# feinanshan/TDNet

Measured on AMD Instinct MI355X. Metric: frames/sec (td4-psp18, 1024x2048, full-resolution logits), higher is better.
Workload: dtype f32; 1 GPU; td4-psp18, 1024x2048 Cityscapes-shaped synthetic stream, 3-frame feature cache, 1 clip per GPU; parallelism=clip-parallel x1, RCCL weight broadcast only, target_fps_per_gpu=30

## Files before the change

include/tdnet.h:

```cpp
#ifndef TDNET_H
#define TDNET_H

#include <stddef.h>
#include <stdint.h>

#ifdef __cplusplus
extern "C" {
#endif

typedef struct tdnet tdnet_t;

typedef struct tdnet_cfg {
    int32_t model;
    int32_t backbone;
    int32_t nclass;
    int32_t height;
    int32_t width;
    int32_t device;
} tdnet_cfg;

#define TDNET_WINOGRAD_DEFAULT 3
#define TDNET_ATTENTION_DEFAULT 2
#define TDNET_FUSION_LN_STATS 2
#define TDNET_FUSION_LN_IN_HEAD 4
#define TDNET_FUSION_A_DIRECT 32
#define TDNET_FUSION_DMA_LOADERS 8192
#define TDNET_FUSION_DMA_NARROW 32768
#define TDNET_FUSION_STEM_ROWS 65536
#define TDNET_FUSION_CONV_GROUPS 131072
#define TDNET_FUSION_CLS_IN_HEAD 262144
#define TDNET_FUSION_SPLIT_NARROW 524288
#define TDNET_FUSION_LATE_CHAIN 1048576
#define TDNET_FUSION_PPM_FOLD 2097152
#define TDNET_OVERLAP_CHAINS 1
#define TDNET_OVERLAP_LOWREG_TRANSFORMS 2
#define TDNET_OVERLAP_CHAINS_ANY_SIZE 4
#define TDNET_OVERLAP_GEMM_DMA 8
#define TDNET_OVERLAP_VW_SHIFT 4
#define TDNET_OVERLAP_VW_MASK 0x30
#define TDNET_FUSION_DEFAULT (TDNET_FUSION_LN_STATS | TDNET_FUSION_LN_IN_HEAD | TDNET_FUSION_A_DIRECT | TDNET_FUSION_DMA_LOADERS | TDNET_FUSION_DMA_NARROW | \
                              TDNET_FUSION_STEM_ROWS | TDNET_FUSION_CONV_GROUPS | TDNET_FUSION_CLS_IN_HEAD | TDNET_FUSION_SPLIT_NARROW | TDNET_FUSION_LATE_CHAIN | TDNET_FUSION_PPM_FOLD)
#define TDNET_FUSION_MASK TDNET_FUSION_DEFAULT
#define TDNET_OVERLAP_DEFAULT (TDNET_OVERLAP_CHAINS | TDNET_OVERLAP_GEMM_DMA | (2 << TDNET_OVERLAP_VW_SHIFT))
#define TDNET_OVERLAP_MASK (TDNET_OVERLAP_CHAINS | TDNET_OVERLAP_LOWREG_TRANSFORMS | TDNET_OVERLAP_CHAINS_ANY_SIZE | TDNET_OVERLAP_GEMM_DMA | TDNET_OVERLAP_VW_MASK)
typedef struct tdnet_opts {
    int32_t winograd;
    int32_t precision;
    int32_t pipeline;
    int32_t gemm_persistent;
    int32_t reserved0;
    int32_t attention;
    int32_t fusion;
    int32_t overlap;
    int32_t reserved[8];
} tdnet_opts;
void tdnet_opts_default(tdnet_opts* o);

typedef struct tdnet_arch {
    int32_t dilated;
    int32_t multi_grid;
    int32_t reserved[6];
} tdnet_arch;
void tdnet_arch_default(tdnet_arch* a);

int  tdnet_create(const tdnet_cfg* cfg, tdnet_t** out);
int  tdnet_create_opts(const tdnet_cfg* cfg, const tdnet_opts* opts , tdnet_t** out);
int  tdnet_create_arch(const tdnet_cfg* cfg, const tdnet_arch* arch , const tdnet_opts* opts ,
                       tdnet_t** out);
int  tdnet_get_opts(const tdnet_t* h, tdnet_opts* out);
int  tdnet_get_arch(const tdnet_t* h, tdnet_arch* out);
int  tdnet_feature_dims(const tdnet_t* h, int* height, int* width);
void tdnet_destroy(tdnet_t* h);

int  tdnet_set_weight(tdnet_t* h, const char* name, const float* host, size_t count);
int  tdnet_finalize_weights(tdnet_t* h);
int  tdnet_create_shared(const tdnet_t* weights_of, const tdnet_opts* opts , tdnet_t** out);
int  tdnet_warmup(tdnet_t* h, void* stream);
// ... 81 lines not shown
```

tdnet_amd/_capi.py:

```python
import ctypes
import os

_HERE = os.path.dirname(os.path.abspath(__file__))
DEFAULT_LIB = os.path.join(_HERE, "lib", "libtdnet_hip.so")
TEST_LIB = os.path.join(_HERE, "lib", "libtdnet_hip_test.so")

c_float_p = ctypes.POINTER(ctypes.c_float)
c_void_p = ctypes.c_void_p


class TdnetCfg(ctypes.Structure):
    _fields_ = [("model", ctypes.c_int32), ("backbone", ctypes.c_int32), ("nclass", ctypes.c_int32),
                ("height", ctypes.c_int32), ("width", ctypes.c_int32), ("device", ctypes.c_int32)]


class TdnetOpts(ctypes.Structure):
    _fields_ = [("winograd", ctypes.c_int32), ("precision", ctypes.c_int32), ("pipeline", ctypes.c_int32),
                ("gemm_persistent", ctypes.c_int32), ("reserved0", ctypes.c_int32), ("attention", ctypes.c_int32),
                ("fusion", ctypes.c_int32), ("overlap", ctypes.c_int32), ("reserved", ctypes.c_int32 * 8)]

    def as_dict(self):
        return {k: getattr(self, k) for k, _ in self._fields_ if not k.startswith("reserved")}


# ... 106 lines not shown
    "tdnet_op_conv1x1_rows": (ctypes.c_int, [c_void_p, ctypes.c_int, ctypes.c_int, ctypes.c_int, c_void_p, c_void_p, ctypes.c_int, ctypes.c_int,
                                             c_opts_p, ctypes.c_int, ctypes.c_int, c_void_p, c_void_p]),
    "tdnet_op_maxpool": (ctypes.c_int, [c_void_p, ctypes.c_int, ctypes.c_int, ctypes.c_int, ctypes.c_int, c_void_p, c_void_p]),
    "tdnet_op_stem_f16": (ctypes.c_int, [c_void_p, ctypes.c_int, ctypes.c_int, c_void_p, c_void_p, ctypes.c_int, c_void_p, c_void_p]),
    "tdnet_op_stem": (ctypes.c_int, [c_void_p, ctypes.c_int, ctypes.c_int, c_void_p, c_void_p, c_opts_p, c_void_p, c_void_p]),
    "tdnet_op_attention": (ctypes.c_int, [c_void_p, c_void_p, c_void_p, c_void_p, c_void_p, ctypes.c_int, ctypes.c_int,
                                          ctypes.c_int, ctypes.c_int, c_void_p, c_void_p, c_void_p, c_void_p, c_void_p]),
    "tdnet_op_layernorm_hw": (ctypes.c_int, [c_void_p, ctypes.c_int, ctypes.c_int, c_void_p, c_void_p, c_void_p, c_void_p]),
    "tdnet_op_layernorm_hw_f16": (ctypes.c_int, [c_void_p, ctypes.c_int, ctypes.c_int, c_void_p, c_void_p, c_void_p, c_void_p]),
    "tdnet_op_ppm": (ctypes.c_int, [c_void_p, ctypes.c_int, ctypes.c_int, c_void_p, c_void_p, ctypes.c_int, ctypes.c_int,
                                    c_void_p, c_void_p]),
    "tdnet_op_upsample": (ctypes.c_int, [c_void_p, ctypes.c_int, ctypes.c_int, ctypes.c_int, ctypes.c_int, ctypes.c_int,
                                         c_void_p, c_void_p]),
    "tdnet_op_stem_image": (ctypes.c_long, [c_void_p, c_void_p, ctypes.c_int, ctypes.c_int, ctypes.c_int, ctypes.c_int, ctypes.POINTER(ctypes.c_double),
                                            ctypes.POINTER(ctypes.c_double), ctypes.c_int, c_void_p, ctypes.c_size_t, c_void_p]),
    "tdnet_op_stem_image_nv12": (ctypes.c_long, [c_void_p, ctypes.c_int, ctypes.c_int, ctypes.c_int, ctypes.c_size_t, ctypes.c_int, ctypes.c_int, ctypes.c_int,
                                                 ctypes.POINTER(ctypes.c_double), ctypes.POINTER(ctypes.c_double), ctypes.c_int, c_void_p, ctypes.c_size_t, c_void_p]),
    "tdnet_op_stem_image_view": (ctypes.c_long, [c_void_p, c_view_p, ctypes.c_int, ctypes.c_int, ctypes.POINTER(ctypes.c_double), ctypes.POINTER(ctypes.c_double),
                                                 ctypes.c_int, c_void_p, ctypes.c_size_t, c_void_p]),
    "tdnet_op_overlay_view": (ctypes.c_int, [c_void_p] + [ctypes.c_int] * 5 + [c_void_p, c_void_p, c_view_p, c_void_p, ctypes.c_int, c_void_p, c_void_p]),
    "tdnet_op_upsample_argmax": (ctypes.c_int, [c_void_p, ctypes.c_int, ctypes.c_int, ctypes.c_int, ctypes.c_int, ctypes.c_int, c_void_p, c_void_p, c_void_p]),
    "tdnet_op_upsample_argmax_rgb": (ctypes.c_int, [c_void_p] + [ctypes.c_int] * 7 + [c_void_p, ctypes.c_int, c_void_p, c_void_p, c_void_p]),
    "tdnet_op_overlay": (ctypes.c_int, [c_void_p] + [ctypes.c_int] * 5 + [c_void_p, c_void_p] + [ctypes.c_int] * 4 + [ctypes.c_size_t, ctypes.c_int, c_void_p, ctypes.c_int,
                                        c_void_p, c_void_p]),
    "tdnet_op_upsample_argmax_score": (ctypes.c_int, [c_void_p] + [ctypes.c_int] * 5 + [c_void_p] * 6),
    "tdnet_op_upsample_argmax_conf": (ctypes.c_int, [c_void_p] + [ctypes.c_int] * 5 + [c_void_p, c_void_p, ctypes.c_int, ctypes.c_int, c_void_p, c_void_p]),
    "tdnet_op_nearest_index": (ctypes.c_int, [ctypes.c_int, ctypes.c_int, c_void_p]),
    "tdnet_op_enc_first": (ctypes.c_int, [c_void_p] + [ctypes.c_int] * 4 + [c_void_p] * 4 + [ctypes.c_int] + [c_void_p] * 4 + [ctypes.c_int] + [c_void_p] * 5),
    "tdnet_op_conv1x1_src2_null": (ctypes.c_int, [c_void_p, ctypes.c_int, ctypes.c_int, ctypes.c_int, c_void_p, c_void_p, ctypes.c_int, ctypes.c_int,
                                                  c_void_p, ctypes.c_int, c_opts_p, ctypes.c_int, c_void_p, c_void_p]),
    "tdnet_op_classifier": (ctypes.c_int, [c_void_p, ctypes.c_int, ctypes.c_int, c_void_p, c_void_p, ctypes.c_int, c_void_p, c_void_p]),
    "tdnet_op_head_cls": (ctypes.c_int, [c_void_p, ctypes.c_int, ctypes.c_int, ctypes.c_int, c_void_p, c_void_p, ctypes.c_int, ctypes.c_int,
                                         c_void_p, c_void_p, ctypes.c_int, c_opts_p, ctypes.c_int, c_void_p, c_void_p]),
}


class Lib:

    def __init__(self, path=DEFAULT_LIB, test_symbols=False):
        if not os.path.exists(path):
            raise TdnetError("HIP library not found: %s -- build it with `python -c 'import __graft_entry__ as g; g.build()'` "
                             "(hipcc --offload-arch=gfx950); there is no CPU fallback" % path)
        self.path = path
        if path in (DEFAULT_LIB, TEST_LIB):
            import torch
        self.dll = ctypes.CDLL(path)
        for name, (res, args) in list(SYMBOLS.items()) + (list(TEST_SYMBOLS.items()) if test_symbols else []):
            fn = getattr(self.dll, name)
            fn.restype = res
            fn.argtypes = args
            setattr(self, name, fn)

    def opts(self, **kw):
        o = TdnetOpts()
        self.tdnet_opts_default(ctypes.byref(o))
        for k, v in kw.items():
            if k not in dict(TdnetOpts._fields_) or k.startswith("reserved"):
                raise TypeError("unknown tdnet_opts field %r" % k)
            if v is not None:
                setattr(o, k, int(v))
        return o

    def arch(self, dilated=True, multi_grid=True):
        a = TdnetArch()
        self.tdnet_arch_default(ctypes.byref(a))
        a.dilated, a.multi_grid = int(bool(dilated)), int(bool(multi_grid))
# ... 25 lines not shown
```

tdnet_amd/csrc/td_frame.h:

```cpp
#pragma once
#include "td_launch.h"

static int free_slot(tdnet* n) {
    for (int i = 0; i < (int)n->slots.size(); ++i) {
        bool used = i == n->pending_slot;
        for (int f : n->fifo) used |= f == i;
        if (!used) return i;
    }
    return -1;
}
static void fifo_commit(tdnet* n, int slot) {
    n->fifo.push_back(slot);
    if ((int)n->fifo.size() > n->FIFO) n->fifo.erase(n->fifo.begin());
    n->last_slot = slot;
}

static int launch_chain(tdnet* n, PathLayers& L, hipStream_t s, float* vp, int e0, int e1, int e2) {
    const int DV = n->DV;
    hipStream_t c = n->side;
    TD_HIP(hipEventRecord(n->ev_fork, s));
    TD_HIP(hipStreamWaitEvent(c, n->ev_fork, 0));
    if (probe_skip() & 2) { TD_HIP(hipEventRecord(n->ev_join, c)); return 0; }
    if (n->P == 4) {
        const CacheSlot &c0 = n->slots[e0], &c1 = n->slots[e1], &c2 = n->slots[e2];
        TD_TRY(run_conv(n, L.atn[0].fc, c0.v, 1, n->Lk, nullptr, vp, c));
        const bool sl = DV == 512 && n->Lk <= 8192;
        if (run_attention(n, c1.q, c0.k, vp, L.atn[0].d_bias, c1.v, n->Lk, n->Lk, DV, n->chain_a, c, n->opts.attention, nullptr, nullptr, sl)) return -1;
        TD_TRY(run_conv(n, L.atn[1].fc, n->chain_a, 1, n->Lk, nullptr, vp, c));
        if (run_attention(n, c2.q, c1.k, vp, L.atn[1].d_bias, c2.v, n->Lk, n->Lk, DV, n->chain_b, c, n->opts.attention, nullptr, nullptr, sl)) return -1;
        TD_TRY(run_conv(n, L.atn[2].fc, n->chain_b, 1, n->Lk, nullptr, vp, c));
    } else {
        TD_TRY(run_conv(n, L.atn[0].fc, n->slots[e0].v, 1, n->Lk, nullptr, vp, c));
    }
    if (n->vt16) {
        prof_begin(n, 2, false, 0, c);
        if (n->opts.precision >= 2) attn_prepare_vt_b3(vp, n->Lk, DV, reinterpret_cast<unsigned short*>(n->vt16), c);
        else attn_prepare_vt_h(vp, n->Lk, DV, n->vt16, c);
        prof_end(n, c);
    }
    TD_HIP(hipEventRecord(n->ev_join, c));
    return 0;
}
static int launch_chain_now(tdnet* n, PathLayers& L, hipStream_t s) {
    return launch_chain(n, L, s, n->vp, n->fifo[0], n->P == 4 ? n->fifo[1] : -1, n->P == 4 ? n->fifo[2] : -1);
}
static int run_ds_rows(tdnet* n, const ConvLayer& L, const float* in, int H, int W, float* out, int ny, int cy, hipStream_t s) {
    if (L.route != CR_GEMM1X1) return td_fail("internal: downsample conv cannot run on image rows");
// ... 62 lines not shown
        const bool last16 = n->act16 && &B == &L.blocks.back();
        if (B.bott) {
            TD_TRY(run_conv(n, B.c1, n->bx, ch, cw, nullptr, n->bt, s));
            TD_TRY(run_conv(n, B.c2, n->bt, ch, cw, nullptr, n->bu, s, &oh, &ow));
            const float* res = n->bx;
            if (B.has_ds) { TD_TRY(run_conv(n, B.ds, n->bx, ch, cw, nullptr, n->br, s)); res = n->br; }
            TD_TRY(run_conv(n, B.c3, n->bu, oh, ow, res, last16 ? n->br : n->bx, s));
        } else {
            const float* res = n->bx;
            if (B.has_ds) {
                const ConvCall both[2] = {{&B.c1, n->bx, ch, cw, n->bt}, {&B.ds, n->bx, ch, cw, n->br}};
                TD_TRY(run_conv_group(n, n->opts, both, 2, s, &oh, &ow));
                res = n->br;
            } else TD_TRY(run_conv(n, B.c1, n->bx, ch, cw, nullptr, n->bt, s, &oh, &ow));
            TD_TRY(run_conv(n, B.c2, n->bt, oh, ow, res, last16 ? n->br : n->bx, s));
        }
        ch = oh; cw = ow;
    }
    float* c4 = n->c4 = n->seg_block >= 0 ? n->seg_x.back() : n->act16 ? n->br : n->bx;
    if (n->cfg.model == 1) {
        run_ppm(n, c4, n->h, n->w, n->C, n->C, n->C / 4, L.d_ppm_w, L.d_ppm_b, 0, n->rowpart, n->pooled, n->ppmfeat, n->z, s);
        TD_TRY(run_conv(n, L.head3, n->z, n->h, n->w, nullptr, n->headmid, s));
        TD_TRY(run_classifier(n, n->headmid, n->Lq, n->MID, n->cfg.nclass, L.d_cls_w, L.d_cls_b, n->lowres, s));
        return n->failed ? -1 : 0;
    }
    const int XS = n->C / 2, FS = n->C / 8;
    const ConvLayer* const firstL[3] = {&L.enc_v, &L.enc_q0, &L.enc_k0};
    const PpmFoldArgs fold = n->enc_fold ? ppm_fold_args(firstL, n->fold_g, n->ppmfeat, XS, FS) : PpmFoldArgs();
    run_ppm(n, c4, n->h, n->w, n->C, XS, FS, L.d_ppm_w, L.d_ppm_b, L.pid, n->rowpart, n->pooled, n->ppmfeat, n->z, s, n->enc_fold ? &fold : nullptr);
    n->z_pending = n->enc_fold;
    n->z_path = (int)(&L - &n->paths[0]);
    const int slot = free_slot(n);
    if (slot < 0) return td_fail("internal: no free cache slot");
    CacheSlot& cs = n->slots[slot];
    const ConvCall first[3] = {{&L.enc_v, n->z, n->h, n->w, n->v_cur}, {&L.enc_q0, n->z, n->h, n->w, n->q1}, {&L.enc_k0, n->z, n->h, n->w, n->k1}};
    const ConvCall second[2] = {{&L.enc_q1, n->q1, n->h, n->w, n->q_cur}, {&L.enc_k1, n->k1, n->hk, n->wk, cs.k}};
    if (n->enc_fold) {
        float* const outs[3] = {n->v_cur, n->q1, n->k1};
        for (int i = 0; i < 3; ++i)
            TD_TRY(run_conv_src2(n, *firstL[i], c4 + L.pid * XS, n->C, XS / 32, XS / 32 + TD_PPM_BASIS / 32, n->ppm_basis, TD_PPM_BASIS, n->fold_g[i], n->h, n->w, nullptr, outs[i], s));
    } else
    TD_TRY(run_conv_group(n, n->opts, first, 3, s));
    TD_TRY(run_conv_group(n, n->opts, second, 2, s));
    prof_begin(n, 2, false, 0, s);
    launch_cache_subsample(n->q_cur, cs.q, 64, n->v_cur, cs.v, DV, n->w, n->hk, n->wk, s);
    prof_end(n, s);
    n->pending_slot = slot;
    return n->failed ? -1 : 0;
}

static int finish_frame(tdnet* n, PathLayers& L, bool steady, hipStream_t s) {
    const int DV = n->DV;
    const float* feat = n->v_cur;
    int stats_nstr = 0;
    n->feat_is_vcur = !steady;
    if (steady) {
        TD_HIP(hipStreamWaitEvent(s, n->ev_join, 0));
        const CacheSlot& ck = n->slots[n->fifo[n->FIFO - 1]];
        const AtnLayer& A = L.atn[n->P == 4 ? 2 : 0];
        stats_nstr = (n->opts.fusion & TDNET_FUSION_LN_STATS) ? attn_strips(n->Lq, DV) : 0;
        if (run_attention(n, n->q_cur, ck.k, n->vp, A.d_bias, n->v_cur, n->Lq, n->Lk, DV, n->feat, s, n->opts.attention,
                          stats_nstr ? n->ln_part : nullptr, nullptr, false, n->vt16 != nullptr, n->opts.precision >= 2)) return -1;
        feat = n->feat;
    }
    const bool ln_in_head = (n->opts.fusion & TDNET_FUSION_LN_IN_HEAD) && L.head3.wino;
    const bool ln16 = L.head3.in16;
    run_layernorm(n, feat, n->Lq, DV, L.d_ln_g, L.d_ln_b, n->ln_part, n->ln_mean, n->ln_rstd, ln_in_head ? nullptr : n->ln, s, stats_nstr, ln16);
    n->ln_pending = ln_in_head || ln16;
    n->ln_path = (int)(&L - &n->paths[0]);
    const bool cls_in_head = (n->opts.fusion & TDNET_FUSION_CLS_IN_HEAD) && L.head3.wino && L.head3.chunks == 1 && wino_out_cls_supports(n->MID, n->cfg.nclass);
    const ClsArgs ca = {L.d_cls_w, L.d_cls_b, n->lowres, n->cfg.nclass};
    if (ln_in_head) {
        const LnFuse lf = {n->ln_mean, n->ln_rstd, L.d_ln_g, L.d_ln_b};
        TD_TRY(run_conv(n, L.head3, feat, n->h, n->w, nullptr, n->headmid, s, nullptr, nullptr, &lf, cls_in_head ? &ca : nullptr));
    } else
    TD_TRY(run_conv(n, L.head3, n->ln, n->h, n->w, nullptr, n->headmid, s, nullptr, nullptr, nullptr, cls_in_head ? &ca : nullptr));
    if (!cls_in_head) TD_TRY(run_classifier(n, n->headmid, n->Lq, n->MID, n->cfg.nclass, L.d_cls_w, L.d_cls_b, n->lowres, s));
    if (n->failed) return -1;
    if (n->pending_slot >= 0) {
        const int slot = n->pending_slot;
        n->pending_slot = -1;
        fifo_commit(n, slot);
    }
    return 0;
}

static int frame_checks(tdnet* n, int pos_id, const char* who, const FrameInput* in = nullptr) {
    if (!n->finalized || !n->ws_ready) return td_fail("%s: weights not finalized (the HIP path never runs on random init)", who);
    if (in && in->kind == TD_IMG_U8 && !n->u8.set) return td_fail("%s: the uint8 input is not configured (call tdnet_set_input_u8 first)", who);
    if (pos_id < 0 || pos_id >= n->P) return td_fail("%s: pos_id %d out of range 0..%d", who, pos_id, n->P - 1);
    return 0;
}

static void rejoin_streams(tdnet* n, hipStream_t s) {
    for (hipStream_t c : {n->side, n->chain2}) {
        if (!c) continue;
        hipEvent_t& e = c == n->side ? n->ev_join : n->ev_cjoin;
        if (e && hipEventRecord(e, c) == hipSuccess) (void)hipStreamWaitEvent(s, e, 0);
    }
}

static int streams_share_a_queue(hipStream_t a, hipStream_t x, hipEvent_t e0, hipEvent_t e1, hipEvent_t e2, bool* shared) {
    float pair_us = 0.f;
    TD_HIP(td_streams_share_a_queue(a, x, e0, e1, e2, shared, &pair_us));
    if (getenv("TDNET_QUEUE_CHECK_VERBOSE")) fprintf(stderr, "tdnet queue check: spin pair %.1f us\n", pair_us);
    return 0;
}
static int place_chain_stream(tdnet* n, hipStream_t s, bool explicit_call = false) {
    if (!n->chain2 || std::find(n->placed_for.begin(), n->placed_for.end(), (void*)s) != n->placed_for.end()) return 0;
    if (!explicit_call && td_stream_is_capturing(s)) return 0;
    n->placed_for.push_back((void*)s);
    if (getenv("TDNET_NO_QUEUE_CHECK")) return 0;
    if (n->placed_for.size() > 8 || n->retired_streams.size() >= 12) return 0;
    hipEvent_t e0 = nullptr, e1 = nullptr, e2 = nullptr;
    TD_HIP(hipEventCreate(&e0)); TD_HIP(hipEventCreate(&e1)); TD_HIP(hipEventCreate(&e2));
    int rc = 0;
    for (int attempt = 0; attempt < 6 && n->retired_streams.size() < 12; ++attempt) {
        bool shared = false;
        if ((rc = streams_share_a_queue(s, n->chain2, e0, e1, e2, &shared)) != 0 || !shared) break;
        hipStream_t fresh = nullptr;
        if (hipStreamCreateWithFlags(&fresh, hipStreamNonBlocking) != hipSuccess) break;
        n->retired_streams.push_back(n->chain2);
        n->chain2 = fresh;
        n->chain_replaced++;
    }
    hipEventDestroy(e0); hipEventDestroy(e1); hipEventDestroy(e2);
    return rc;
// ... 28 lines not shown
```

tdnet_amd/csrc/td_handle.h:

```cpp
#pragma once
#include "../../include/tdnet.h"
#include "td_device.h"
#include "td_conv.h"
#include "td_conv_h.h"
#include "td_conv_hd.h"
#include "td_conv_ad.h"
#include "td_wino.h"
#include "td_gemm.h"
#include "td_gemm_dma.h"
#include "td_gemm_b3.h"
#include "td_conv_ad_b3.h"
#include "td_attn.h"
#include "td_attn_h.h"
#include "td_attn_b3.h"
#include "td_misc.h"
#include "td_ingest.h"
#include "td_out.h"
#include "td_score.h"
#include "td_conf.h"

#include <cmath>
#include <cstdarg>
#include <cstdio>
#include <algorithm>
// ... 89 lines not shown
    CR_STEM_H,
    CR_CONV_H,
    CR_CONV_DMA,
    CR_WINO
};
enum GemmKernel {
    GK_CONV,
    GK_PERSISTENT,
    GK_DMA,
    GK_B3
};
struct ConvLayer {
    int Cin = 0, Cout = 0, KS = 1, stride = 1, dil = 1, pad = 0, act = 0;
    bool stem = false;
    ConvRoute route = CR_IGEMM;
    GemmKernel gemm = GK_CONV;
    bool in16 = false, out16 = false;
    int rh = 0;
    bool rowimg_off = false;
    int pers = 1;
    int chunks = 1;
    int vw = 0;
    int wino = 0;
    float* d_zero = nullptr;
    ConvTile tile = CT_128x128;
    int CoutPad = 0, nsteps = 0;
    float* d_wp = nullptr;
    float* d_bias = nullptr;
    bool h16() const { return route == CR_STEM_H || route == CR_CONV_H || route == CR_CONV_DMA; }
    bool stem_rows() const { return route == CR_ADIRECT_ROWS || route == CR_ADIRECT_ROWS_B3; }
    double flops_per_pixel() const { return 2.0 * Cout * (stem ? 3.0 * KS * KS : (double)Cin * KS * KS); }
};

static_assert(TDNET_FUSION_DEFAULT == 4169766 && TDNET_FUSION_MASK == 4169766 && TDNET_OVERLAP_DEFAULT == 41 && TDNET_OVERLAP_MASK == 0x3f,
              "the named option bits of include/tdnet.h must add up to the documented values");
static tdnet_opts opts_or_default(const tdnet_opts* o) {
    tdnet_opts d;
    tdnet_opts_default(&d);
    if (!o) return d;
    d = *o;
    d.winograd = d.winograd <= 0 ? 0 : (d.winograd == 2 || d.winograd >= 4) ? 4 : 3;
    d.precision = d.precision < 0 ? 0 : d.precision > 3 ? 1 : d.precision;
    d.pipeline = d.pipeline ? 1 : 0;
    d.gemm_persistent = d.gemm_persistent < 0 ? 0 : d.gemm_persistent;
    d.attention = d.attention < 0 ? 0 : d.attention > 2 ? 2 : d.attention;
    d.fusion &= TDNET_FUSION_MASK;
    d.overlap = d.overlap < 0 ? 0 : d.overlap & TDNET_OVERLAP_MASK;
    if ((d.overlap & TDNET_OVERLAP_VW_MASK) == TDNET_OVERLAP_VW_MASK) d.overlap &= ~TDNET_OVERLAP_VW_MASK;
    d.reserved0 = 0;
    for (int& r : d.reserved) r = 0;
    return d;
}

struct BlockLayers { ConvLayer c1, c2, c3, ds; bool has_ds = false, bott = false; };
struct AtnLayer { ConvLayer fc; float* d_bias = nullptr; };
struct PathLayers {
    ConvLayer stem, stem2, stem3;
    std::vector<BlockLayers> blocks;
    float* d_ppm_w = nullptr; float* d_ppm_b = nullptr;
    ConvLayer enc_v, enc_q0, enc_q1, enc_k0, enc_k1;
    std::vector<AtnLayer> atn;
    float* d_ln_g = nullptr; float* d_ln_b = nullptr;
    ConvLayer head3;
    float* d_cls_w = nullptr; float* d_cls_b = nullptr;
    int pid = 0;
};
struct CacheSlot { float* q = nullptr; float* k = nullptr; float* v = nullptr; };
// ... 78 lines not shown
    tdnet_opts opts;
    int P = 0, DV = 0, MID = 0, FIFO = 0, C = 512, SC = 64;
    bool deep = false;
    int H = 0, W = 0, H1 = 0, W1 = 0, H2 = 0, W2 = 0, h = 0, w = 0, hk = 0, wk = 0, Lq = 0, Lk = 0;
    std::vector<BlockSpec>& bspec;
    std::map<std::string, std::vector<float>>& sd;
    std::map<std::string, size_t>& expected;
    bool& finalized;
    std::vector<PathLayers>& paths;
    int& seg_block; int& seg_conv;
    bool& act16;
    double& flops_frame;
    bool ws_ready = false;
    size_t ws_bytes = 0;
    float *img4 = nullptr, *s1 = nullptr, *s1b = nullptr, *bx = nullptr, *bt = nullptr, *br = nullptr, *bu = nullptr;
    float *rowpart = nullptr, *pooled = nullptr, *ppmfeat = nullptr, *z = nullptr;
    float *v_cur = nullptr, *q1 = nullptr, *q_cur = nullptr, *k1 = nullptr;
    float *vp = nullptr, *chain_a = nullptr, *chain_b = nullptr, *feat = nullptr;
    float *ln_part = nullptr, *ln_mean = nullptr, *ln_rstd = nullptr, *ln = nullptr;
    float *headmid = nullptr, *lowres = nullptr, *stage_tmp = nullptr, *logits_tmp = nullptr;
    float *wino_v = nullptr, *wino_m = nullptr;
    size_t wino_v_floats = 0, wino_m_floats = 0;
    size_t stage_tmp_floats = 0;
    std::vector<CacheSlot> slots;
    std::vector<int> fifo;
    int last_slot = -1;
    int pending_slot = -1;
    int pending_pos = -1;
    hipStream_t side = nullptr;
    hipEvent_t ev_fork = nullptr, ev_join = nullptr;
    hipStream_t chain2 = nullptr;
    hipEvent_t ev_cfork = nullptr, ev_cjoin = nullptr;
    float *wino_v2 = nullptr, *wino_m2 = nullptr;
    std::vector<float*> seg_t, seg_r, seg_x;
    std::vector<hipStream_t> probe_streams;
    std::vector<hipStream_t> retired_streams;
    std::vector<void*> placed_for;
    int chain_replaced = 0;
    float* c4 = nullptr;
    _Float16* vt16 = nullptr;
    bool ln_pending = false;
    bool enc_fold = false;
    float* ppm_basis = nullptr;
    float* fold_g[3] = {nullptr, nullptr, nullptr};
    bool z_pending = false;
    int z_path = 0;
    int ln_path = 0;
    bool feat_is_vcur = false;
    bool failed = false;
    bool prof = false;
    std::vector<ProfRec> recs;
    size_t nrec = 0;
    U8Input u8;
    RgbOutput rgb;
    OverlayOutput overlay;
    ScoreOutput score;
    int min_conf = 0, reject_label = 255;
    int launches = 0;

    explicit tdnet(TdWeights* w)
        : wt(w), bspec(w->bspec), sd(w->sd), expected(w->expected), finalized(w->finalized), paths(w->paths), seg_block(w->seg_block),
          seg_conv(w->seg_conv), act16(w->act16), flops_frame(w->flops_frame) {}
    tdnet(const tdnet&) = delete;
    tdnet& operator=(const tdnet&) = delete;
};

// ... 300 lines not shown
```

tdnet_amd/csrc/td_model.hip:

```cpp
#include "td_frame.h"

extern "C" const char* tdnet_last_error(void) { return g_err; }
#ifndef TDNET_SRC_HASH
#define TDNET_SRC_HASH "unstamped"
#endif
extern "C" const char* tdnet_version(void) { return "tdnet_amd 0.3 (gfx950, fp32 MFMA) tdnet-src-hash:" TDNET_SRC_HASH; }
extern "C" void tdnet_opts_default(tdnet_opts* o) {
    if (!o) return;
    memset(o, 0, sizeof(*o));
    o->winograd = TDNET_WINOGRAD_DEFAULT;
    o->precision = 0;
    o->pipeline = 1;
    o->gemm_persistent = 1;
    o->attention = TDNET_ATTENTION_DEFAULT;
    o->fusion = TDNET_FUSION_DEFAULT;
    o->overlap = TDNET_OVERLAP_DEFAULT;
}
extern "C" void tdnet_arch_default(tdnet_arch* a) {
    if (!a) return;
    memset(a, 0, sizeof(*a));
    a->dilated = 1;
    a->multi_grid = 1;
}
extern "C" int tdnet_create(const tdnet_cfg* cfg, tdnet_t** out) { return tdnet_create_opts(cfg, nullptr, out); }
// ... 83 lines not shown
    tdnet* n = new tdnet(weights_of->wt);
    n->wt->refs.fetch_add(1, std::memory_order_relaxed);
    set_geometry(n, &weights_of->cfg);
    n->opts = weights_of->opts;
    if (init_handle(n)) { tdnet_destroy(n); return -1; }
    *out = n;
    return 0;
}

extern "C" void tdnet_destroy(tdnet_t* n) {
    if (!n) return;
    TD_ON_DEVICE(n);
    for (float* q : {n->img4, n->s1, n->s1b, n->bx, n->bt, n->br, n->bu, n->rowpart, n->pooled, n->ppmfeat, n->z, n->v_cur, n->q1, n->q_cur,
                     n->k1, n->vp, n->chain_a, n->chain_b, n->feat, n->ln_part, n->ln_mean, n->ln_rstd, n->ln, n->headmid,
                     n->lowres, n->stage_tmp, n->logits_tmp, n->wino_v, n->wino_m, n->ppm_basis, n->fold_g[0], n->fold_g[1], n->fold_g[2]})
        if (q) hipFree(q);
    for (auto& s : n->slots) { if (s.q) hipFree(s.q); if (s.k) hipFree(s.k); if (s.v) hipFree(s.v); }
    for (auto& r : n->recs) { hipEventDestroy(r.e0); hipEventDestroy(r.e1); }
    if (n->vt16) hipFree(n->vt16);
    u8_free(n->u8);
    rgb_free(n->rgb);
    overlay_free(n->overlay);
    score_free(n->score);
    for (float* q : {n->wino_v2, n->wino_m2}) if (q) hipFree(q);
    for (auto* v : {&n->seg_t, &n->seg_r, &n->seg_x}) for (float* q : *v) if (q) hipFree(q);
    if (n->chain2) hipStreamDestroy(n->chain2);
    for (hipStream_t x : n->probe_streams) hipStreamDestroy(x);
    for (hipStream_t x : n->retired_streams) hipStreamDestroy(x);
    if (n->ev_cfork) hipEventDestroy(n->ev_cfork);
    if (n->ev_cjoin) hipEventDestroy(n->ev_cjoin);
    if (n->side) hipStreamDestroy(n->side);
    if (n->ev_fork) hipEventDestroy(n->ev_fork);
    if (n->ev_join) hipEventDestroy(n->ev_join);
    TdWeights* wt = n->wt;
    delete n;
    if (wt->refs.fetch_sub(1, std::memory_order_acq_rel) == 1) {
        for (auto& p : wt->paths) free_path(p);
        delete wt;
    }
}

extern "C" int tdnet_set_weight(tdnet_t* n, const char* name, const float* host, size_t count) {
    if (!n || !name || !host) return td_fail("tdnet_set_weight: null argument");
    if (n->finalized) return td_fail("tdnet_set_weight: weights already finalized");
    auto it = n->expected.find(name);
    if (it == n->expected.end()) return td_fail("Unexpected key in state_dict: \"%s\"", name);
    if (it->second != count) return td_fail("size mismatch for %s: expected %zu elements, got %zu", name, it->second, count);
    const std::string s = name;
    if (s.find(".fc.weight") != std::string::npos && s.compare(0, 10, "pretrained") == 0) return 0;
    if (s.find(".fc.bias") != std::string::npos && s.compare(0, 10, "pretrained") == 0) return 0;
    if (s.size() > 19 && s.compare(s.size() - 19, 19, "num_batches_tracked") == 0) { n->sd[s] = {0.f}; return 0; }
    n->sd[s].assign(host, host + count);
    return 0;
}
extern "C" int tdnet_finalize_weights(tdnet_t* n) {
    if (!n) return td_fail("tdnet_finalize_weights: null handle");
    if (n->finalized) return td_fail("tdnet_finalize_weights: already finalized");
    TD_ON_DEVICE(n, -1);
    TD_TRY(finalize_block(n));
    return init_handle(n);
}
extern "C" int tdnet_warmup(tdnet_t* n, void* stream) {
    if (!n) return td_fail("tdnet_warmup: null handle");
    if (!n->finalized || !n->ws_ready) return td_fail("tdnet_warmup: weights not finalized");
    TD_ON_DEVICE(n, -1);
    return place_chain_stream(n, (hipStream_t)stream, true);
// ... 8 lines not shown
extern "C" int tdnet_streams_share_queue(void* stream_a, void* stream_b, int* shared) {
    if (!shared) return td_fail("tdnet_streams_share_queue: shared is NULL");
    *shared = 0;
    if (stream_a == stream_b) { *shared = 1; return 0; }
    hipEvent_t e0 = nullptr, e1 = nullptr, e2 = nullptr;
    if (hipEventCreate(&e0) != hipSuccess || hipEventCreate(&e1) != hipSuccess || hipEventCreate(&e2) != hipSuccess) {
        if (e0) hipEventDestroy(e0);
        if (e1) hipEventDestroy(e1);
        return td_fail("tdnet_streams_share_queue: hipEventCreate failed");
    }
    bool sh = false;
    const int rc = streams_share_a_queue((hipStream_t)stream_a, (hipStream_t)stream_b, e0, e1, e2, &sh);
    hipEventDestroy(e0); hipEventDestroy(e1); hipEventDestroy(e2);
    *shared = sh ? 1 : 0;
    return rc;
}

struct LaunchCount {
    tdnet* n; long l0;
    explicit LaunchCount(tdnet* n_) : n(n_), l0(td_launch_count) {}
    ~LaunchCount() { n->launches = (int)(td_launch_count - l0); }
};
struct FrameSource { const FrameInput* img; int pos_id; };
static int propagate_lowres(tdnet* n, hipStream_t s);
static int frame_out(tdnet* n, const FrameSource& src, const FrameOutput& out, void* stream, const char* who) {
    TD_ON_DEVICE(n, -1);
    TD_TRY(output_configured(n, out.kind, who));
    LaunchCount count_(n);
    hipStream_t s = (hipStream_t)stream;
    if (src.img ? forward_lowres(n, *src.img, src.pos_id, s, who) : propagate_lowres(n, s)) return -1;
    if (src.img) prof_begin(n, 2, false, 0, s);
    const int rc = emit_output(n, out, s, who);
    if (src.img) prof_end(n, s);
    TD_HIP(hipGetLastError());
    return rc;
}
static int frame_out(tdnet* n, const FrameInput& img, int pos_id, const FrameOutput& out, void* stream, const char* who) {
    return frame_out(n, FrameSource{&img, pos_id}, out, stream, who);
}
static inline FrameInput frame_input_u8(const tdnet* n, const uint8_t* img) { return FrameInput{img, TD_IMG_U8, &n->u8}; }
extern "C" int tdnet_forward(tdnet_t* n, const float* img, int pos_id, float* logits, void* stream) {
    if (!n || !img || !logits) return td_fail("tdnet_forward: null argument");
    return frame_out(n, frame_input_f32(img), pos_id, FrameOutput{OUT_LOGITS, logits}, stream, "tdnet_forward");
}
extern "C" int tdnet_forward_u8(tdnet_t* n, const uint8_t* img, int pos_id, float* logits, void* stream) {
    if (!n || !img || !logits) return td_fail("tdnet_forward_u8: null argument");
    return frame_out(n, frame_input_u8(n, img), pos_id, FrameOutput{OUT_LOGITS, logits}, stream, "tdnet_forward_u8");
}
extern "C" int tdnet_argmax(tdnet_t* n, const float* logits, int32_t* labels, void* stream) {
    if (!n || !logits || !labels) return td_fail("tdnet_argmax: null argument");
    TD_ON_DEVICE(n, -1);
    launch_argmax(logits, n->cfg.nclass, (long)n->H * n->W, labels, (hipStream_t)stream);
    TD_HIP(hipGetLastError());
    return 0;
}
extern "C" int tdnet_argmax_u8(tdnet_t* n, const float* logits, uint8_t* labels, void* stream) {
    if (!n || !logits || !labels) return td_fail("tdnet_argmax_u8: null argument");
    TD_ON_DEVICE(n, -1);
    TD_TRY(launch_argmax_u8(logits, n->cfg.nclass, (long)n->H * n->W, labels, (hipStream_t)stream));
    TD_HIP(hipGetLastError());
    return 0;
}
extern "C" int tdnet_forward_labels(tdnet_t* n, const float* img, int pos_id, int32_t* labels, void* stream) {
    if (!n || !img || !labels) return td_fail("tdnet_forward_labels: null argument");
    return frame_out(n, frame_input_f32(img), pos_id, FrameOutput{OUT_LABELS_I32, labels}, stream, "tdnet_forward");
}
// ... 159 lines not shown
extern "C" int tdnet_set_confidence(tdnet_t* n, int min_conf, int reject_label) {
    if (!n) return td_fail("tdnet_set_confidence: null handle");
    if (min_conf < 0 || min_conf > 255) return td_fail("tdnet_set_confidence: min_conf = %d must be in 0..255", min_conf);
    if (reject_label < 0 || reject_label > 255) return td_fail("tdnet_set_confidence: reject_label = %d must be in 0..255", reject_label);
    n->min_conf = min_conf;
    n->reject_label = reject_label;
    return 0;
}
extern "C" int tdnet_forward_labels_conf(tdnet_t* n, const float* img, int pos_id, uint8_t* labels, uint8_t* conf, void* stream) {
    if (!n || !img || !conf) return td_fail("tdnet_forward_labels_conf: null argument");
    return frame_out(n, frame_input_f32(img), pos_id, FrameOutput{OUT_CONF, labels, nullptr, conf}, stream, "tdnet_forward_labels_conf");
}
extern "C" int tdnet_forward_u8_labels_conf(tdnet_t* n, const uint8_t* img, int pos_id, uint8_t* labels, uint8_t* conf, void* stream) {
    if (!n || !img || !conf) return td_fail("tdnet_forward_u8_labels_conf: null argument");
    return frame_out(n, frame_input_u8(n, img), pos_id, FrameOutput{OUT_CONF, labels, nullptr, conf}, stream, "tdnet_forward_u8_labels_conf");
}
extern "C" int tdnet_logits_conf(tdnet_t* n, const float* logits, uint8_t* labels, uint8_t* conf, void* stream) {
    if (!n || !logits || !conf) return td_fail("tdnet_logits_conf: null argument");
    if (!n->finalized || !n->ws_ready) return td_fail("tdnet_logits_conf: weights not finalized");
    TD_ON_DEVICE(n, -1);
    TD_TRY(launch_logits_conf_u8(logits, n->cfg.nclass, (long)n->H * n->W, labels, conf, n->min_conf, n->reject_label, (hipStream_t)stream));
    TD_HIP(hipGetLastError());
    return 0;
}
static int encode_impl(tdnet* n, const FrameInput& img, int pos_id, void* stream, const char* who) {
    TD_ON_DEVICE(n, -1);
    if (frame_checks(n, pos_id, who, &img)) return -1;
    if (n->cfg.model == 1) return td_fail("%s: pspnet has no temporal state; use tdnet_forward", who);
    if (n->pending_slot >= 0) return td_fail("%s: the previous encoded frame has not been propagated", who);
    n->nrec = 0;
    n->failed = false;
    TD_TRY(place_chain_stream(n, (hipStream_t)stream));
    LaunchCount count_(n);
    if (encode_frame(n, n->paths[pos_id], img, (hipStream_t)stream)) {
        rejoin_streams(n, (hipStream_t)stream);
        n->pending_slot = n->pending_pos = -1;
        return -1;
    }
    n->pending_pos = pos_id;
    TD_HIP(hipGetLastError());
    return 0;
}
extern "C" int tdnet_encode(tdnet_t* n, const float* img, int pos_id, void* stream) {
    if (!n || !img) return td_fail("tdnet_encode: null argument");
    return encode_impl(n, frame_input_f32(img), pos_id, stream, "tdnet_encode");
}
extern "C" int tdnet_encode_u8(tdnet_t* n, const uint8_t* img, int pos_id, void* stream) {
    if (!n || !img) return td_fail("tdnet_encode_u8: null argument");
    return encode_impl(n, frame_input_u8(n, img), pos_id, stream, "tdnet_encode_u8");
}
static int propagate_lowres(tdnet* n, hipStream_t s) {
    if (n->pending_slot < 0) return td_fail("tdnet_propagate: no encoded frame (call tdnet_encode first)");
    PathLayers& L = n->paths[n->pending_pos];
    const bool steady = (int)n->fifo.size() >= n->FIFO;
    if ((steady && launch_chain_now(n, L, s)) || finish_frame(n, L, steady, s)) { rejoin_streams(n, s); n->pending_slot = n->pending_pos = -1; return -1; }
    return 0;
}
static const FrameSource pending_frame = {nullptr, -1};
extern "C" int tdnet_propagate(tdnet_t* n, float* logits, void* stream) {
    if (!n || !logits) return td_fail("tdnet_propagate: null argument");
    return frame_out(n, pending_frame, FrameOutput{OUT_LOGITS, logits}, stream, "tdnet_propagate");
}
extern "C" int tdnet_propagate_labels(tdnet_t* n, int32_t* labels, void* stream) {
    if (!n || !labels) return td_fail("tdnet_propagate_labels: null argument");
    return frame_out(n, pending_frame, FrameOutput{OUT_LABELS_I32, labels}, stream, "tdnet_propagate_labels");
}
extern "C" int tdnet_propagate_labels_u8(tdnet_t* n, uint8_t* labels, void* stream) {
// ... 146 lines not shown
```

tdnet_amd/csrc/td_weights.h:

```cpp
#pragma once
#include "td_handle.h"

constexpr int RH_FRAME = -1;
constexpr int RH_BY_SIZE = -2;

static int plan_dma_form(const ConvLayer& c, long M, const tdnet_opts& o) {
    const bool narrow = (o.fusion & TDNET_FUSION_DMA_NARROW) != 0, same3 = c.KS == 3 && c.stride == 1 && c.pad == c.dil;
    if (!conv_dma_supports(c.Cin, c.Cout, c.KS, c.tile)) return CD_NONE;
    if (c.Cout == 64 && c.CoutPad == 128 && same3 && narrow) return CD_128_N;
    if (c.Cout < 128) return CD_NONE;
    const int rh = conv_dma_pick_rh(M, c.Cout, c.CoutPad % 256 == 0);
    if (narrow && same3 && M <= 16384 && c.Cout <= 256) return c.Cout <= 128 ? CD_128_N : CD_192_N;
    if (o.fusion & TDNET_FUSION_DMA_LOADERS) return rh == CD_128 ? CD_128_P : rh == CD_192 ? CD_192_P : rh;
    return rh;
}

static int plan_conv(ConvLayer& L, int Cout, int Cin, int KS, int stride, int dil, int act, bool stem, long M, const tdnet_opts& o,
                     int forced_tile = -1, int chunks = 1, bool in16 = false, bool out16 = false, int rh = RH_FRAME, bool rowimg_off = false) {
    L = ConvLayer();
    L.Cin = stem ? 4 : Cin; L.Cout = Cout; L.KS = KS; L.stride = stride; L.dil = dil; L.act = act; L.stem = stem;
    L.pad = stem ? KS / 2 : dil * (KS / 2);
    L.pers = o.gemm_persistent;
    L.rowimg_off = rowimg_off;
    if (!stem && Cin % 32 != 0) return td_fail("conv: Cin=%d is not a multiple of 32", Cin);
// ... 456 lines not shown
    {
        static std::atomic<bool> told{false};
        const char* q = getenv("GPU_MAX_HW_QUEUES");
        if (!getenv("TDNET_QUIET") && (!q || atoi(q) > 3) && !told.exchange(true)) {
            fprintf(stderr, "tdnet: GPU_MAX_HW_QUEUES is %s; export GPU_MAX_HW_QUEUES=2 before the HIP runtime starts -- with more hardware queues "
                            "alive in the process this handle's streams are time-sliced (275 -> 185 frames/s measured behind an RCCL communicator)\n", q ? q : "not set");
        }
    }
    {
        AllocScope count_(&n->ws_bytes);
        if (alloc_workspace(n)) return -1;
    }
    TD_HIP(hipDeviceSynchronize());
#ifdef TDNET_TIMING_PROBES
    if (const char* e = getenv("TDNET_PROBE_EXTRA_STREAMS")) {
        for (int i = 0, k = atoi(e); i < k && i < 16; ++i) {
            hipStream_t x = nullptr;
            if (hipStreamCreateWithFlags(&x, hipStreamNonBlocking) == hipSuccess) n->probe_streams.push_back(x);
        }
    }
#endif
    {
        int least = 0, greatest = 0;
        TD_HIP(hipDeviceGetStreamPriorityRange(&least, &greatest));
        TD_HIP(hipStreamCreateWithPriority(&n->side, hipStreamNonBlocking, least));
    }
    if (n->seg_block >= 0) {
        TD_HIP(hipStreamCreateWithFlags(&n->chain2, hipStreamNonBlocking));
        TD_HIP(hipEventCreateWithFlags(&n->ev_cfork, hipEventDisableTiming));
        TD_HIP(hipEventCreateWithFlags(&n->ev_cjoin, hipEventDisableTiming));
    }
    TD_HIP(hipEventCreateWithFlags(&n->ev_fork, hipEventDisableTiming));
    TD_HIP(hipEventCreateWithFlags(&n->ev_join, hipEventDisableTiming));
    n->ws_ready = true;
    return 0;
}

static double frame_flops(const tdnet* n) {
    const PathLayers& L = n->paths[0];
    double f = L.stem.flops_per_pixel() * n->H1 * n->W1;
    if (n->deep) f += (L.stem2.flops_per_pixel() + L.stem3.flops_per_pixel()) * n->H1 * n->W1;
    int ch = n->H2, cw = n->W2;
    for (size_t i = 0; i < L.blocks.size(); ++i) {
        const BlockSpec& s = n->bspec[i];
        const int oh = out_size(ch, 3, s.stride, s.dil1, s.dil1), ow = out_size(cw, 3, s.stride, s.dil1, s.dil1);
        const double M = (double)oh * ow;
        if (s.bott) f += (double)ch * cw * L.blocks[i].c1.flops_per_pixel() + M * (L.blocks[i].c2.flops_per_pixel() + L.blocks[i].c3.flops_per_pixel());
        else f += M * (L.blocks[i].c1.flops_per_pixel() + L.blocks[i].c2.flops_per_pixel());
        if (s.ds) f += M * L.blocks[i].ds.flops_per_pixel();
        ch = oh; cw = ow;
    }
    const double C = n->C;
    if (n->cfg.model == 1)
        return f + 2.0 * 50 * (C / 4) * C * 4 / 4 + (double)n->Lq * (2.0 * 2 * C * 9 * n->MID + 2.0 * n->MID * n->cfg.nclass);
    const double Lq = n->Lq, Lk = n->Lk, DV = n->DV;
    f += 2.0 * (1 + 4 + 9 + 36) * (C / 4) * C;
    f += Lq * (2.0 * C * DV + 2.0 * C * 64 + 2.0 * 64 * 64);
    f += Lk * (2.0 * C * DV + 2 * (2.0 * C * 64 + 2.0 * 64 * 64));
    if (n->P == 4) {
        f += 2 * (2.0 * Lk * Lk * (64 + DV) + 2.0 * Lk * DV * DV);
        f += 2.0 * Lq * Lk * (64 + DV) + 2.0 * Lq * DV * DV;
    } else {
        f += 2.0 * Lq * Lk * (64 + DV) + 2.0 * Lq * DV * DV;
    }
    f += Lq * (2.0 * DV * 9 * n->MID + 2.0 * n->MID * n->cfg.nclass);
    return f;
// ... 2 lines not shown
```

Measured before the change: 290.7 frames/s.

## Overlap cache-entry key conv and subsample on side stream during head

Adds a new default-on overlap bit that defers the key-encoder convolutions and the cache subsample of the current frame onto a low-priority side stream. That work is forked after the attention/head starts and joined after output emission. The aim is to hide these small, independent launches behind the main-stream head work instead of serialising them. The cost is extra event record/wait pairs and new fork/join state whose error paths must be handled correctly.

```diff
diff --git a/include/tdnet.h b/include/tdnet.h
--- a/include/tdnet.h
+++ b/include/tdnet.h
@@ -38,11 +38,13 @@
 #define TDNET_OVERLAP_GEMM_DMA 8
 #define TDNET_OVERLAP_VW_SHIFT 4
 #define TDNET_OVERLAP_VW_MASK 0x30
+#define TDNET_OVERLAP_SIDE_BRANCHES 256
 #define TDNET_FUSION_DEFAULT (TDNET_FUSION_LN_STATS | TDNET_FUSION_LN_IN_HEAD | TDNET_FUSION_A_DIRECT | TDNET_FUSION_DMA_LOADERS | TDNET_FUSION_DMA_NARROW | \
                               TDNET_FUSION_STEM_ROWS | TDNET_FUSION_CONV_GROUPS | TDNET_FUSION_CLS_IN_HEAD | TDNET_FUSION_SPLIT_NARROW | TDNET_FUSION_LATE_CHAIN | TDNET_FUSION_PPM_FOLD)
 #define TDNET_FUSION_MASK TDNET_FUSION_DEFAULT
-#define TDNET_OVERLAP_DEFAULT (TDNET_OVERLAP_CHAINS | TDNET_OVERLAP_GEMM_DMA | (2 << TDNET_OVERLAP_VW_SHIFT))
-#define TDNET_OVERLAP_MASK (TDNET_OVERLAP_CHAINS | TDNET_OVERLAP_LOWREG_TRANSFORMS | TDNET_OVERLAP_CHAINS_ANY_SIZE | TDNET_OVERLAP_GEMM_DMA | TDNET_OVERLAP_VW_MASK)
+#define TDNET_OVERLAP_DEFAULT (TDNET_OVERLAP_CHAINS | TDNET_OVERLAP_GEMM_DMA | (2 << TDNET_OVERLAP_VW_SHIFT) | TDNET_OVERLAP_SIDE_BRANCHES)
+#define TDNET_OVERLAP_MASK (TDNET_OVERLAP_CHAINS | TDNET_OVERLAP_LOWREG_TRANSFORMS | TDNET_OVERLAP_CHAINS_ANY_SIZE | TDNET_OVERLAP_GEMM_DMA | TDNET_OVERLAP_VW_MASK | \
+                            TDNET_OVERLAP_SIDE_BRANCHES)
 typedef struct tdnet_opts {
     int32_t winograd;
     int32_t precision;
diff --git a/tdnet_amd/_capi.py b/tdnet_amd/_capi.py
--- a/tdnet_amd/_capi.py
+++ b/tdnet_amd/_capi.py
@@ -162,6 +162,7 @@
     "tdnet_op_classifier": (ctypes.c_int, [c_void_p, ctypes.c_int, ctypes.c_int, c_void_p, c_void_p, ctypes.c_int, c_void_p, c_void_p]),
     "tdnet_op_head_cls": (ctypes.c_int, [c_void_p, ctypes.c_int, ctypes.c_int, ctypes.c_int, c_void_p, c_void_p, ctypes.c_int, ctypes.c_int,
                                          c_void_p, c_void_p, ctypes.c_int, c_opts_p, ctypes.c_int, c_void_p, c_void_p]),
+    "tdnet_test_side_branches_late": (ctypes.c_int, [c_void_p, ctypes.c_int]),
 }
 
 
diff --git a/tdnet_amd/csrc/td_frame.h b/tdnet_amd/csrc/td_frame.h
--- a/tdnet_amd/csrc/td_frame.h
+++ b/tdnet_amd/csrc/td_frame.h
@@ -13,6 +13,48 @@
     n->fifo.push_back(slot);
     if ((int)n->fifo.size() > n->FIFO) n->fifo.erase(n->fifo.begin());
     n->last_slot = slot;
+}
+
+static bool side_branch_on(const tdnet* n) { return n->side && (n->opts.overlap & TDNET_OVERLAP_SIDE_BRANCHES) && !(probe_skip() & 16); }
+
+struct EncCalls {
+    ConvCall first[3], second[2];
+    bool g1, g2;
+    EncCalls(const tdnet* n, const PathLayers& L, int slot)
+        : first{{&L.enc_v, n->z, n->h, n->w, n->v_cur}, {&L.enc_q0, n->z, n->h, n->w, n->q1}, {&L.enc_k0, n->z, n->h, n->w, n->k1}},
+          second{{&L.enc_q1, n->q1, n->h, n->w, n->q_cur}, {&L.enc_k1, n->k1, n->hk, n->wk, n->slots[slot].k}},
+          g1(!n->enc_fold && conv_group_same_form(n->opts, first, 3)), g2(conv_group_same_form(n->opts, second, 2)) {}
+};
+static int run_enc_first(tdnet* n, const PathLayers& L, const EncCalls& E, int i, hipStream_t s) {
+    const ConvCall& c = E.first[i];
+    if (!n->enc_fold) return run_conv(n, *c.L, c.in, c.H, c.W, nullptr, c.out, s);
+    const int XS = n->C / 2;
+    return run_conv_src2(n, *c.L, n->c4 + L.pid * XS, n->C, XS / 32, XS / 32 + TD_PPM_BASIS / 32, n->ppm_basis, TD_PPM_BASIS, n->fold_g[i], n->h, n->w, nullptr, c.out, s);
+}
+static int launch_cache_entry(tdnet* n, PathLayers& L, int slot, hipStream_t c) {
+    const EncCalls E(n, L, slot);
+    const CacheSlot& cs = n->slots[slot];
+    if (!E.g1) TD_TRY(run_enc_first(n, L, E, 2, c));
+    if (!E.g2) TD_TRY(run_conv(n, L.enc_k1, n->k1, n->hk, n->wk, nullptr, cs.k, c));
+    prof_begin(n, 2, false, 0, c);
+    launch_cache_subsample(n->q_cur, cs.q, 64, n->v_cur, cs.v, n->DV, n->w, n->hk, n->wk, c);
+    prof_end(n, c);
+    return 0;
+}
+static int fork_side_branch(tdnet* n, hipStream_t s, bool at_join = false) {
+    if (n->a_pending != 2 || (n->branches_late && !at_join)) return 0;
+    TD_HIP(hipEventRecord(n->ev_afork, s));
+    TD_HIP(hipStreamWaitEvent(n->side, n->ev_afork, 0));
+    n->a_pending = 1;
+    return launch_cache_entry(n, n->paths[n->a_path], n->a_slot, n->side);
+}
+static int join_side_branch(tdnet* n, hipStream_t s) {
+    if (!n->a_pending) return 0;
+    TD_TRY(fork_side_branch(n, s, true));
+    n->a_pending = 0;
+    TD_HIP(hipEventRecord(n->ev_adone, n->side));
+    TD_HIP(hipStreamWaitEvent(s, n->ev_adone, 0));
+    return 0;
 }
 
 static int launch_chain(tdnet* n, PathLayers& L, hipStream_t s, float* vp, int e0, int e1, int e2) {
@@ -141,19 +183,19 @@
     n->z_path = (int)(&L - &n->paths[0]);
     const int slot = free_slot(n);
     if (slot < 0) return td_fail("internal: no free cache slot");
-    CacheSlot& cs = n->slots[slot];
-    const ConvCall first[3] = {{&L.enc_v, n->z, n->h, n->w, n->v_cur}, {&L.enc_q0, n->z, n->h, n->w, n->q1}, {&L.enc_k0, n->z, n->h, n->w, n->k1}};
-    const ConvCall second[2] = {{&L.enc_q1, n->q1, n->h, n->w, n->q_cur}, {&L.enc_k1, n->k1, n->hk, n->wk, cs.k}};
-    if (n->enc_fold) {
-        float* const outs[3] = {n->v_cur, n->q1, n->k1};
-        for (int i = 0; i < 3; ++i)
-            TD_TRY(run_conv_src2(n, *firstL[i], c4 + L.pid * XS, n->C, XS / 32, XS / 32 + TD_PPM_BASIS / 32, n->ppm_basis, TD_PPM_BASIS, n->fold_g[i], n->h, n->w, nullptr, outs[i], s));
-    } else
-    TD_TRY(run_conv_group(n, n->opts, first, 3, s));
-    TD_TRY(run_conv_group(n, n->opts, second, 2, s));
-    prof_begin(n, 2, false, 0, s);
-    launch_cache_subsample(n->q_cur, cs.q, 64, n->v_cur, cs.v, DV, n->w, n->hk, n->wk, s);
-    prof_end(n, s);
+    const CacheSlot& cs = n->slots[slot];
+    const EncCalls E(n, L, slot);
+    const bool branch = side_branch_on(n);
+    if (E.g1) TD_TRY(run_conv_group(n, n->opts, E.first, 3, s));
+    else for (int i = 0; i < (branch ? 2 : 3); ++i) TD_TRY(run_enc_first(n, L, E, i, s));
+    if (E.g2 || !branch) TD_TRY(run_conv_group(n, n->opts, E.second, 2, s));
+    else TD_TRY(run_conv(n, L.enc_q1, n->q1, n->h, n->w, nullptr, n->q_cur, s));
+    if (branch) { n->a_slot = slot; n->a_path = n->z_path; n->a_pending = 2; }
+    else {
+        prof_begin(n, 2, false, 0, s);
+        launch_cache_subsample(n->q_cur, cs.q, 64, n->v_cur, cs.v, DV, n->w, n->hk, n->wk, s);
+        prof_end(n, s);
+    }
     n->pending_slot = slot;
     return n->failed ? -1 : 0;
 }
@@ -172,6 +214,7 @@
                           stats_nstr ? n->ln_part : nullptr, nullptr, false, n->vt16 != nullptr, n->opts.precision >= 2)) return -1;
         feat = n->feat;
     }
+    TD_TRY(fork_side_branch(n, s));
     const bool ln_in_head = (n->opts.fusion & TDNET_FUSION_LN_IN_HEAD) && L.head3.wino;
     const bool ln16 = L.head3.in16;
     run_layernorm(n, feat, n->Lq, DV, L.d_ln_g, L.d_ln_b, n->ln_part, n->ln_mean, n->ln_rstd, ln_in_head ? nullptr : n->ln, s, stats_nstr, ln16);
@@ -202,6 +245,7 @@
 }
 
 static void rejoin_streams(tdnet* n, hipStream_t s) {
+    n->a_pending = 0;
     for (hipStream_t c : {n->side, n->chain2}) {
         if (!c) continue;
         hipEvent_t& e = c == n->side ? n->ev_join : n->ev_cjoin;
diff --git a/tdnet_amd/csrc/td_handle.h b/tdnet_amd/csrc/td_handle.h
--- a/tdnet_amd/csrc/td_handle.h
+++ b/tdnet_amd/csrc/td_handle.h
@@ -145,7 +145,7 @@
     double flops_per_pixel() const { return 2.0 * Cout * (stem ? 3.0 * KS * KS : (double)Cin * KS * KS); }
 };
 
-static_assert(TDNET_FUSION_DEFAULT == 4169766 && TDNET_FUSION_MASK == 4169766 && TDNET_OVERLAP_DEFAULT == 41 && TDNET_OVERLAP_MASK == 0x3f,
+static_assert(TDNET_FUSION_DEFAULT == 4169766 && TDNET_FUSION_MASK == 4169766 && TDNET_OVERLAP_DEFAULT == 297 && TDNET_OVERLAP_MASK == 0x13f,
               "the named option bits of include/tdnet.h must add up to the documented values");
 static tdnet_opts opts_or_default(const tdnet_opts* o) {
     tdnet_opts d;
@@ -290,6 +290,10 @@
     hipStream_t chain2 = nullptr;
     hipEvent_t ev_cfork = nullptr, ev_cjoin = nullptr;
     float *wino_v2 = nullptr, *wino_m2 = nullptr;
+    hipEvent_t ev_afork = nullptr, ev_adone = nullptr;
+    int a_pending = 0;
+    int a_slot = -1, a_path = 0;
+    bool branches_late = false;
     std::vector<float*> seg_t, seg_r, seg_x;
     std::vector<hipStream_t> probe_streams;
     std::vector<hipStream_t> retired_streams;
diff --git a/tdnet_amd/csrc/td_model.hip b/tdnet_amd/csrc/td_model.hip
--- a/tdnet_amd/csrc/td_model.hip
+++ b/tdnet_amd/csrc/td_model.hip
@@ -139,6 +139,7 @@
     if (n->side) hipStreamDestroy(n->side);
     if (n->ev_fork) hipEventDestroy(n->ev_fork);
     if (n->ev_join) hipEventDestroy(n->ev_join);
+    for (hipEvent_t e : {n->ev_afork, n->ev_adone}) if (e) hipEventDestroy(e);
     TdWeights* wt = n->wt;
     delete n;
     if (wt->refs.fetch_sub(1, std::memory_order_acq_rel) == 1) {
@@ -213,6 +214,7 @@
     if (src.img) prof_begin(n, 2, false, 0, s);
     const int rc = emit_output(n, out, s, who);
     if (src.img) prof_end(n, s);
+    if (join_side_branch(n, s)) { rejoin_streams(n, s); return -1; }
     TD_HIP(hipGetLastError());
     return rc;
 }
@@ -438,7 +440,7 @@
     n->failed = false;
     TD_TRY(place_chain_stream(n, (hipStream_t)stream));
     LaunchCount count_(n);
-    if (encode_frame(n, n->paths[pos_id], img, (hipStream_t)stream)) {
+    if (encode_frame(n, n->paths[pos_id], img, (hipStream_t)stream) || fork_side_branch(n, (hipStream_t)stream) || join_side_branch(n, (hipStream_t)stream)) {
         rejoin_streams(n, (hipStream_t)stream);
         n->pending_slot = n->pending_pos = -1;
         return -1;
diff --git a/tdnet_amd/csrc/td_weights.h b/tdnet_amd/csrc/td_weights.h
--- a/tdnet_amd/csrc/td_weights.h
+++ b/tdnet_amd/csrc/td_weights.h
@@ -512,6 +512,7 @@
     }
     TD_HIP(hipEventCreateWithFlags(&n->ev_fork, hipEventDisableTiming));
     TD_HIP(hipEventCreateWithFlags(&n->ev_join, hipEventDisableTiming));
+    for (hipEvent_t* e : {&n->ev_afork, &n->ev_adone}) TD_HIP(hipEventCreateWithFlags(e, hipEventDisableTiming));
     n->ws_ready = true;
     return 0;
 }
```

New measurement: 291.3 frames/s, median of 4. About the same (+0.2%).
